# sacs-epfl/decentralized-learning-simulator

Hardware: AMD Instinct MI355X
Metric: device-resident GB/s, N-way weighted model-tensor reduce; 1/2/4/8 MI355X (higher is better)
Workload: dtype f32

## Files before the change

decentralized-learning-simulator_amd/csrc/dispatch.hpp:

```cpp
#pragma once

#include <hip/hip_runtime.h>

#include <algorithm>
#include <cmath>
#include <cstdint>
#include <cstdlib>
#include <cstring>
#include <type_traits>
#include <vector>

#include "dlsim.h"
#include "wreduce_kernels.hpp"
#include "chunk_mean_kernels.hpp"
#include "ab_env.hpp"


namespace dlsim_host __attribute__((visibility("hidden"))) {

int fail(int code, const char* fmt, ...) __attribute__((format(printf, 2, 3)));
int hip_fail(hipError_t e, const char* what);

constexpr int kVpt = 4;
constexpr size_t kBatchSmallBytes = size_t{1} << 20;
// ... 349 lines not shown
                     dim3(dlsim::kBlock), 0, st, s);
  return hipGetLastError();
}

template <class Op, int K, int VPT>
hipError_t launch_batch_fixed(const dlsim::BatchSlots& s, int n, unsigned blocks, hipStream_t st) {
  if constexpr (K > max_fixed_fan_in<Op>()) {
    return launch_batch_nf<Op, 0, VPT>(s, blocks, st);
  } else {
    if (n == K) return launch_batch_nf<Op, K, VPT>(s, blocks, st);
    return launch_batch_fixed<Op, K + 1, VPT>(s, n, blocks, st);
  }
}

template <class Op>
hipError_t launch_batch(const int* fan_in, const size_t* in_off, const void* const* in, const float* w,
                        const float* divs, void* const* outs, const size_t* nelem, int t0, int t1,
                        hipStream_t st) {
  dlsim::BatchSlots s;
  std::memset(&s, 0, sizeof(s));
  const int vpt = batch_vpt<Op>(nelem, t0, t1);
  const size_t tile = static_cast<size_t>(dlsim::kBlock) * vpt;
  uint32_t blocks = 0;
  int ptrs = 0;
  bool uniform = true;
  for (int t = t0; t < t1; ++t) {
    const int k = t - t0;
    const size_t nvec = nelem[t] / Op::E;
    s.out[k] = outs[t];
    s.nvec[k] = nvec;
    s.nelem[k] = nelem[t];
    s.block_start[k] = blocks - static_cast<uint32_t>(k);
    s.ptr_off[k] = static_cast<uint32_t>(ptrs);
    s.fan_in[k] = static_cast<uint32_t>(fan_in[t]);
    s.div[k] = divs ? divs[t] : 1.0f;
    for (int i = 0; i < fan_in[t]; ++i) {
      s.p[ptrs + i] = in[in_off[t] + i];
      s.w[ptrs + i] = w[in_off[t] + i];
    }
    ptrs += fan_in[t];
    blocks += static_cast<uint32_t>(nvec / tile + 1);
    uniform = uniform && fan_in[t] == fan_in[t0];
  }
  s.ntasks = t1 - t0;
  s.block_start[t1 - t0] = blocks - static_cast<uint32_t>(t1 - t0);
  if (vpt == 1) {
    if (uniform) return launch_batch_fixed<Op, 1, 1>(s, fan_in[t0], blocks, st);
    return launch_batch_nf<Op, 0, 1>(s, blocks, st);
  }
  if (uniform) return launch_batch_fixed<Op, 1, 4>(s, fan_in[t0], blocks, st);
  return launch_batch_nf<Op, 0, 4>(s, blocks, st);
}

template <class Op>
int run_batched(int b, const int* fan_in, const void* const* in, const float* w, void* const* outs,
                const size_t* nelem, hipStream_t st, const float* divs = nullptr) {
  std::vector<size_t> off(static_cast<size_t>(b) + 1, 0);
  for (int t = 0; t < b; ++t) off[t + 1] = off[t] + static_cast<size_t>(fan_in[t]);
  if (cross_task_overlap(b, fan_in, in, outs, nelem, Op::kBytes)) {
    for (int t = 0; t < b; ++t) {
      int rc = run<Op>(in + off[t], fan_in[t], w + off[t], outs[t], nelem[t], st, divs ? divs[t] : 1.0f);
      if (rc != DLSIM_OK) return rc;
    }
    return DLSIM_OK;
  }
  auto batchable = [&](int t) {
    if (nelem[t] == 0 || fan_in[t] > 16) return false;
    if (nelem[t] * Op::kBytes > kMaxLaunchOutBytes) return false;
    if (use_defer<Op>(fan_in[t], nelem[t])) return false;
    if (!aligned16(outs[t])) return false;
    for (int i = 0; i < fan_in[t]; ++i)
      if (!aligned16(in[off[t] + i])) return false;
    return true;
  };
  std::vector<int> group;
  for (int t = 0; t < b; ++t) {
    if (batchable(t)) {
      group.push_back(t);
      continue;
    }
    if (nelem[t] == 0) continue;
    int rc = run<Op>(in + off[t], fan_in[t], w + off[t], outs[t], nelem[t], st, divs ? divs[t] : 1.0f);
    if (rc != DLSIM_OK) return rc;
  }
  std::vector<const void*> ins;
  std::vector<float> ws, dv;
  std::vector<void*> os;
  std::vector<size_t> ne, ioff;
  std::vector<int> fi;
  for (int t : group) {
    ioff.push_back(ins.size());
    for (int i = 0; i < fan_in[t]; ++i) {
      ins.push_back(in[off[t] + i]);
      ws.push_back(w[off[t] + i]);
    }
    os.push_back(outs[t]);
    ne.push_back(nelem[t]);
    fi.push_back(fan_in[t]);
    dv.push_back(divs ? divs[t] : 1.0f);
  }
  const int g = static_cast<int>(group.size());
  const size_t tile1 = dlsim::kBlock;
  int t0 = 0;
  while (t0 < g) {
    int t1 = t0, ptrs = 0;
    uint64_t blocks = 0;
    while (t1 < g && t1 - t0 < dlsim::kBatchMaxTasks && ptrs + fi[t1] <= dlsim::kBatchMaxPtrs &&
           blocks + ne[t1] / Op::E / tile1 + 1 < 0x7fffffffull) {
      ptrs += fi[t1];
      blocks += ne[t1] / Op::E / tile1 + 1;
      ++t1;
    }
    hipError_t e = launch_batch<Op>(fi.data(), ioff.data(), ins.data(), ws.data(), dv.data(), os.data(),
                                    ne.data(), t0, t1, st);
    if (e != hipSuccess) return hip_fail(e, "batched kernel launch");
    t0 = t1;
  }
  return DLSIM_OK;
}

struct TableLayout {
  size_t tasks_off, map_off, ptrs_off, w_off, bytes;
  uint32_t nblocks;
  int vpt;
};

inline size_t round8(size_t x) { return (x + 7) / 8 * 8; }

template <class Op>
// ... 50 lines not shown
    const size_t total = nelem[t] * Op::kBytes;
    if (fan_in[t] > DLSIM_MAX_FUSED_INPUTS || total > kMaxLaunchOutBytes || !aligned16(outs[t]))
      return fail(DLSIM_E_ARG, "task %d cannot be table-batched (fan-in <= %d, 16-B aligned, < 2 GiB)", t,
                  DLSIM_MAX_FUSED_INPUTS);
    const uint32_t nb = task_blocks<Op>(nelem[t], L.vpt);
    tasks[t].out = outs[t];
    tasks[t].nvec = nelem[t] / Op::E;
    tasks[t].nelem = nelem[t];
    tasks[t].block_start = blk - 1;
    tasks[t].ptr_off = off;
    tasks[t].fan_in = static_cast<uint32_t>(fan_in[t]);
    map[t] = static_cast<uint32_t>(t);
    for (uint32_t k = 0; k + 1 < nb; ++k) map[blk + k] = static_cast<uint32_t>(t);
    for (int i = 0; i < fan_in[t]; ++i) {
      if (!aligned16(in[off + i]))
        return fail(DLSIM_E_ARG, "task %d input %d is not 16-byte aligned", t, i);
      ptrs[off + i] = in[off + i];
      ws[off + i] = w[off + i];
    }
    blk += nb - 1;
    off += static_cast<uint32_t>(fan_in[t]);
    uniform = uniform && fan_in[t] == fan_in[0];
  }
  h->uniform_fan_in = uniform ? static_cast<uint32_t>(fan_in[0]) : 0u;
  return DLSIM_OK;
}

template <class Op, int NF, int VPT>
hipError_t launch_table_nf(const void* d_table, uint32_t blocks, hipStream_t st) {
  hipLaunchKernelGGL((dlsim::k_wreduce_batch_table<Op, NF, group_size<Op>(), VPT, kNT, store_policy<Op>(),
                                                    kBatchWave<Op, VPT>>),
                     dim3(blocks), dim3(dlsim::kBlock), 0, st, static_cast<const unsigned char*>(d_table));
  return hipGetLastError();
}

template <class Op, int K, int VPT>
hipError_t launch_table_fixed(const void* d_table, int n, uint32_t blocks, hipStream_t st) {
  if constexpr (K > max_fixed_fan_in<Op>()) {
    return launch_table_nf<Op, 0, VPT>(d_table, blocks, st);
  } else {
    if (n == K) return launch_table_nf<Op, K, VPT>(d_table, blocks, st);
    return launch_table_fixed<Op, K + 1, VPT>(d_table, n, blocks, st);
  }
}

template <class Op>
int table_launch(const void* h_table, const void* d_table, hipStream_t st) {
  const auto* h = static_cast<const dlsim::BatchTableHeader*>(h_table);
  if (h->ntasks == 0) return DLSIM_OK;
  if (h->vpt != 1 && h->vpt != 4)
    return fail(DLSIM_E_ARG, "not a table written by dlsim_batch_table_fill (vectors per lane %u)", h->vpt);
  const int n = static_cast<int>(h->uniform_fan_in);
  hipError_t e;
  if (h->vpt == 1)
    e = n ? launch_table_fixed<Op, 1, 1>(d_table, n, h->nblocks, st) : launch_table_nf<Op, 0, 1>(d_table, h->nblocks, st);
  else
    e = n ? launch_table_fixed<Op, 1, 4>(d_table, n, h->nblocks, st) : launch_table_nf<Op, 0, 4>(d_table, h->nblocks, st);
  if (e != hipSuccess) return hip_fail(e, "table batch launch");
  return DLSIM_OK;
}


inline size_t chunk_mean_ilp_begin(int m, size_t n, int threads, size_t esz = 4, size_t vw = 8) {
  if (n <= 1) return 0;
  const size_t rnd = 128 / esz;
  size_t b = 0, e = n;
  if (!(static_cast<unsigned long long>(m) * n < 32768ULL || threads <= 1)) {
    const size_t tp = static_cast<size_t>(threads) < n ? static_cast<size_t>(threads) : n;
    const size_t cs = (n + tp - 1) / tp;
    for (size_t t = 0; t < tp; ++t) {
      size_t tb = t * cs;
      if (tb >= n) break;
      size_t te = tb + cs < n ? tb + cs : n;
      tb -= tb % rnd;
      if (te != n) te -= te % rnd;
      if (tb < te) {
        b = tb;
        e = te;
      }
    }
  }
  const size_t s1 = e - b;
  return b + (s1 >= vw ? s1 / (4 * vw) * (4 * vw) : s1 / 4 * 4);
}

using CmDefault = dlsim::CmShape<4, true, 8>;
using CmFewRows = dlsim::CmShape<4, true, 4>;
constexpr int kCmFewRowsMax = 6;

constexpr int kCmDeferRMax = 32, kCmDeferU = kDeferU, kCmDeferMinRows = 16;
inline bool chunk_defer_on() {
  static const bool on = [] {
    const char* e = dlsim::ab_getenv("DLSIM_CHUNK_DEFER");
    return !(e && e[0] == '0');
  }();
  return on;
}
inline int chunk_defer_min_m() {
  static const int k = [] {
    const char* e = dlsim::ab_getenv("DLSIM_CHUNK_DEFER_MIN_M");
    return e ? std::atoi(e) : kCmDeferMinRows;
  }();
  return k;
}
constexpr int kCmFixedMinM = 4, kCmFixedMaxM = 15;
inline bool chunk_defer_fixed_on() {
// ... 307 lines not shown
```

decentralized-learning-simulator_amd/csrc/dlsim_abi.hip:

```cpp
#include <hip/hip_runtime.h>

#include <algorithm>
#include <cstdarg>
#include <cstdio>
#include <cstdint>
#include <cstdlib>
#include <cstring>
#include <mutex>
#include <string>
#include <thread>
#include <vector>

#include "abi_common.hpp"
#include "dispatch.hpp"
#include "fanin_checks.hpp"

#include "host_pack.hpp"

namespace dlsim_host __attribute__((visibility("hidden"))) {

template <class F>
int with_policy(int dtype, int mode, F&& f) {
  const bool fast = mode == DLSIM_FAST;
  if (dtype == DLSIM_F32) return fast ? f(dlsim::F32Fast{}) : f(dlsim::F32Exact{});
// ... 1436 lines not shown
            : nullptr;
  }
  if (prev >= 0 && prev != device) (void)hipSetDevice(prev);
  if (!out) return nullptr;
  std::lock_guard<std::mutex> lk(g_pool_mu);
  if (out != p) g_realigned.emplace_back(out, p);
  (contig ? g_pool_contig : g_pool_fallback) += 1;
  g_pool_live += nbytes;
  return out;
}

void dlsim_pool_free(void* d_ptr, size_t nbytes, int device, void* ) {
  if (!d_ptr) return;
  void* base = d_ptr;
  {
    std::lock_guard<std::mutex> lk(g_pool_mu);
    for (size_t i = 0; i < g_realigned.size(); ++i) {
      if (g_realigned[i].first == d_ptr) {
        base = g_realigned[i].second;
        g_realigned.erase(g_realigned.begin() + static_cast<long>(i));
        break;
      }
    }
    g_pool_live -= std::min<unsigned long long>(g_pool_live, nbytes);
  }
  int prev = -1;
  (void)hipGetDevice(&prev);
  if (prev != device) (void)hipSetDevice(device);
  (void)hipFree(base);
  if (prev >= 0 && prev != device) (void)hipSetDevice(prev);
}

void dlsim_pool_stats(unsigned long long* contiguous, unsigned long long* fallback, unsigned long long* live_bytes) {
  std::lock_guard<std::mutex> lk(g_pool_mu);
  if (contiguous) *contiguous = g_pool_contig;
  if (fallback) *fallback = g_pool_fallback;
  if (live_bytes) *live_bytes = g_pool_live;
}

const char* dlsim_last_error(void) { return g_err.c_str(); }

const char* dlsim_kernel_name(int n, size_t n_elems, int dtype, int mode) {
  if (dtype != DLSIM_F32 && dtype != DLSIM_BF16 && dtype != DLSIM_F16) return "";
  if (mode == -1) return with_mean_policy_name(dtype, n, n_elems);
  if (mode != DLSIM_EXACT && mode != DLSIM_FAST) return "";
  const char* name = "";
  with_policy(dtype, mode, [&](auto op) {
    name = kernel_name<decltype(op)>(n, n_elems);
    return 0;
  });
  return name;
}

int dlsim_version(void) { return (1 << 16) | 1; }

}
```

decentralized-learning-simulator_amd/csrc/wreduce_kernels.hpp:

```cpp
#pragma once

#include <hip/hip_runtime.h>
#include <stdint.h>

#include <type_traits>

#pragma clang fp contract(off)

namespace dlsim {

constexpr int kBlock = 256;

typedef uint32_t u32x4 __attribute__((ext_vector_type(4)));
typedef float f32x2 __attribute__((ext_vector_type(2)));
typedef __bf16 bf16x2 __attribute__((ext_vector_type(2)));

__device__ __forceinline__ float bf16_round(float f) {
  uint32_t u = __float_as_uint(f);
  if ((u & 0x7fffffffu) > 0x7f800000u) return __uint_as_float(0x7fc00000u);
  u += 0x7fffu + ((u >> 16) & 1u);
  return __uint_as_float(u & 0xffff0000u);
}

__device__ __forceinline__ void bf16_round2(float& a0, float& a1) {
// ... 673 lines not shown
      defer_rows<Op, S, NF, G, RMAX, U, STP>(*ks, n, o, base, R, nvec);
    }
  } else {
    for (int r = 0; r < R; ++r)
      reduce_tile<Op, S, NF, G, 1, 1, true, STP, kDeferBlock>(s, NF > 0 ? NF : n, o,
                                                              base + static_cast<size_t>(r) * kDeferBlock, nvec);
  }
  if (blockIdx.x == 0) {
    const size_t j = nvec * Op::E + threadIdx.x;
    if (j < nelem) fold_scalar<Op, S>(s, NF > 0 ? NF : n, out, j);
  }
}

template <class Op, class S, int NF, int G, int RMAX, int U, int STP, int RC = 0>
__global__ __launch_bounds__(kDeferBlock) void k_wreduce_defer(const S s, int n, int Rrt, void* __restrict__ out,
                                                               size_t nvec, size_t nelem) {
  defer_body<Op, S, NF, G, RMAX, U, STP, RC>(s, n, Rrt, out, nvec, nelem);
}

template <class Op, class S, int NF, int G, int RMAX, int U, int STP, int RC = 0>
__global__ __launch_bounds__(kDeferBlock) void k_wreduce_defer_pre(size_t nvec, void* __restrict__ out,
                                                                   const void* q0, const void* q1, const void* q2,
                                                                   const void* q3, const void* q4, const S s, int n,
                                                                   int Rrt, size_t nelem) {
  static_assert(NF > 0, "fixed fan-in");
  const PreSlots<S> ps{{q0, q1, q2, q3, q4}, s};
  defer_body<Op, PreSlots<S>, NF, G, RMAX, U, STP, RC>(ps, n, Rrt, out, nvec, nelem);
}

constexpr int kBatchMaxTasks = 32;
constexpr int kBatchMaxPtrs = 192;

struct BatchSlots {
  const void* p[kBatchMaxPtrs];
  float w[kBatchMaxPtrs];
  void* out[kBatchMaxTasks];
  size_t nvec[kBatchMaxTasks];
  size_t nelem[kBatchMaxTasks];
  float div[kBatchMaxTasks];
  uint32_t block_start[kBatchMaxTasks + 1];
  uint32_t ptr_off[kBatchMaxTasks];
  uint32_t fan_in[kBatchMaxTasks];
  int ntasks;
};
static_assert(sizeof(BatchSlots) <= 4096, "kernel arguments");

__device__ __forceinline__ int batch_find_task(const BatchSlots& s, uint32_t f) {
  int t = 0;
#pragma unroll
  for (int j = 1; j < kBatchMaxTasks; ++j) t += (j < s.ntasks && f >= s.block_start[j]) ? 1 : 0;
  return t;
}

struct TaskArgs {
  const BatchSlots& b;
  int off;
  float d;
  __device__ const void* ptr(int i) const { return b.p[off + i]; }
  __device__ float wt(int i) const { return b.w[off + i]; }
  __device__ float divisor() const { return d; }
};

template <class Op, int NF, int G, int VPT, int NT, int STP, bool WAVEMAP = false>
__global__ __launch_bounds__(kBlock) void k_wreduce_batch(const BatchSlots s) {
  const uint32_t bid = blockIdx.x;
  int t = 0;
  uint32_t local = 0;
  if (bid < static_cast<uint32_t>(s.ntasks)) {
    t = static_cast<int>(bid);
  } else {
    const uint32_t f = bid - static_cast<uint32_t>(s.ntasks);
    t = batch_find_task(s, f);
    local = f - s.block_start[t] + 1;
  }
  const TaskArgs a{s, static_cast<int>(s.ptr_off[t]), s.div[t]};
  const int n = NF > 0 ? NF : static_cast<int>(s.fan_in[t]);
  const size_t nvec = s.nvec[t];
  constexpr size_t kTile = static_cast<size_t>(kBlock) * VPT;
  const size_t full = nvec / kTile;
  const OutRef o = make_out<STP>(s.out[t], nvec);
  if (local == 0) {
    if (full * kTile < nvec)
      reduce_tile<Op, TaskArgs, NF, G, VPT, NT, true, STP>(a, n, o, full * kTile + threadIdx.x, nvec);
    const size_t j = nvec * Op::E + threadIdx.x;
    if (j < s.nelem[t]) fold_scalar<Op, TaskArgs>(a, n, s.out[t], j);
    return;
  }
  if constexpr (WAVEMAP) {
    const size_t lane_off = (threadIdx.x >> 6) * 64 * VPT + (threadIdx.x & 63);
    reduce_tile<Op, TaskArgs, NF, G, VPT, NT, false, STP, 64>(a, n, o, (local - 1) * kTile + lane_off, nvec);
  } else {
    reduce_tile<Op, TaskArgs, NF, G, VPT, NT, false, STP>(a, n, o, (local - 1) * kTile + threadIdx.x, nvec);
  }
}

struct BatchTableHeader {
  uint32_t ntasks;
  uint32_t nblocks;
  uint32_t uniform_fan_in;
  uint32_t vpt;
  uint64_t tasks_off;
  uint64_t map_off;
  uint64_t ptrs_off;
  uint64_t w_off;
};

struct BatchTaskDesc {
  void* out;
  uint64_t nvec;
  uint64_t nelem;
  uint32_t block_start;
  uint32_t ptr_off;
  uint32_t fan_in;
  uint32_t reserved;
};

struct TableArgs {
  const void* const* p;
  const float* w;
  __device__ const void* ptr(int i) const { return p[i]; }
  __device__ float wt(int i) const { return w[i]; }
  __device__ float divisor() const { return 1.0f; }
};

template <class Op, int NF, int G, int VPT, int NT, int STP, bool WAVEMAP = false>
__global__ __launch_bounds__(kBlock) void k_wreduce_batch_table(const unsigned char* __restrict__ table) {
  const BatchTableHeader* h = reinterpret_cast<const BatchTableHeader*>(table);
  const uint32_t* map = reinterpret_cast<const uint32_t*>(table + h->map_off);
  const uint32_t t = map[blockIdx.x];
  const BatchTaskDesc d = reinterpret_cast<const BatchTaskDesc*>(table + h->tasks_off)[t];
  const TableArgs a{reinterpret_cast<const void* const*>(table + h->ptrs_off) + d.ptr_off,
                    reinterpret_cast<const float*>(table + h->w_off) + d.ptr_off};
  const int n = NF > 0 ? NF : static_cast<int>(d.fan_in);
  const size_t nvec = d.nvec;
  constexpr size_t kTile = static_cast<size_t>(kBlock) * VPT;
  const size_t full = nvec / kTile;
  const OutRef o = make_out<STP>(d.out, nvec);
  const uint32_t local = blockIdx.x < h->ntasks ? 0u : blockIdx.x - d.block_start;
  if (local == 0) {
    if (full * kTile < nvec)
      reduce_tile<Op, TableArgs, NF, G, VPT, NT, true, STP>(a, n, o, full * kTile + threadIdx.x, nvec);
    const size_t j = nvec * Op::E + threadIdx.x;
    if (j < d.nelem) fold_scalar<Op, TableArgs>(a, n, d.out, j);
    return;
  }
// ... 99 lines not shown
```

decentralized-learning-simulator_amd/dasklearn_amd/_native.py:

```python
from __future__ import annotations

import ctypes
import os
import threading
from typing import Optional, Sequence

import numpy as np

LIB_DIR = os.path.join(os.path.dirname(os.path.abspath(__file__)), "lib")
LIB_PATH = os.path.join(LIB_DIR, "libdlsim_hip.so")

DLSIM_F32 = 0
DLSIM_BF16 = 1
DLSIM_F16 = 2
DLSIM_F64 = 3
DLSIM_EXACT = 0
DLSIM_FAST = 1
MAX_FUSED_INPUTS = 128
DLSIM_E_ARG = -1
DLSIM_E_RCCL = -4
DLSIM_E_PEER = -5
DLSIM_E_DISAGREE = -6
DLSIM_GATHER_NONE = 0
DLSIM_GATHER_BCAST = 1
# ... 10 lines not shown
    "dlsim_wreduce_f64",
    "dlsim_wreduce_tensors",
    "dlsim_wreduce_batched",
    "dlsim_batch_table_bytes",
    "dlsim_batch_table_fill",
    "dlsim_batch_table_launch",
    "dlsim_mean",
    "dlsim_mean_batched",
    "dlsim_chunk_mean_batched",
    "dlsim_chunk_mean_ilp_begin",
    "dlsim_chunk_mean_plan",
    "dlsim_rccl_bind",
    "dlsim_wreduce_sharded",
    "dlsim_wreduce_sharded_f64",
    "dlsim_wreduce_mixed",
    "dlsim_sgd_step",
    "dlsim_sgd_step_tensors",
    "dlsim_sgd_momentum_step",
    "dlsim_sgd_momentum_step_tensors",
    "dlsim_robust_reduce",
    "dlsim_robust_reduce_tensors",
    "dlsim_robust_reduce_batched",
    "dlsim_robust_batch_geometry",
    "dlsim_robust_reduce_tensors_batched",
    "dlsim_robust_nearest_reduce",
    "dlsim_robust_nearest_reduce_tensors",
    "dlsim_pairwise_sqdist",
    "dlsim_pairwise_sqdist_tensors",
    "dlsim_pairdist_geometry",
    "dlsim_pairwise_sqdist_batched",
    "dlsim_pairdist_batch_geometry",
    "dlsim_wreduce_dist_batched",
    "dlsim_reducedist_batch_geometry",
    "dlsim_wreduce_dist",
    "dlsim_wreduce_dist_tensors",
    "dlsim_reducedist_geometry",
    "dlsim_device_alloc",
    "dlsim_device_free",
    "dlsim_pool_alloc",
    "dlsim_pool_free",
    "dlsim_pool_stats",
    "dlsim_sharded_plan_create",
    "dlsim_sharded_plan_run",
    "dlsim_sharded_plan_run_f64",
    "dlsim_sharded_plan_destroy",
    "dlsim_host_wreduce",
    "dlsim_host_wreduce_zc",
    "dlsim_host_wreduce_resident",
    "dlsim_host_chunk_mean",
    "dlsim_host_pack",
    "dlsim_shard_range",
    "dlsim_probe_pattern",
    "dlsim_kernel_name",
    "dlsim_last_error",
    "dlsim_version",
)

_lib = None
_lock = threading.Lock()


class ChunkLaunch(ctypes.Structure):
    _fields_ = [("form", ctypes.c_int), ("mf", ctypes.c_int), ("rows", ctypes.c_int), ("bpt", ctypes.c_int),
                ("grid", ctypes.c_uint), ("ntasks", ctypes.c_int), ("first_task", ctypes.c_int)]


CHUNK_FORMS = ("tiled_few", "tiled", "table", "defer_rf4", "defer_rf8", "defer_m")


class DlsimError(RuntimeError):

    def __init__(self, fn: str, rc: int, msg: str):
        super().__init__(f"{fn} failed (rc={rc}): {msg}")
        self.rc = rc


def load() -> ctypes.CDLL:
    global _lib
    if _lib is not None:
        return _lib
    with _lock:
        if _lib is not None:
            return _lib
        if not os.path.exists(LIB_PATH):
            raise ImportError(
                f"HIP extension not built: {LIB_PATH} is missing. Run "
                "`python -c 'import __graft_entry__ as g; g.build()'` at the repo root.")
        lib = ctypes.CDLL(LIB_PATH)
        vp, sz, i = ctypes.c_void_p, ctypes.c_size_t, ctypes.c_int
        lib.dlsim_wreduce.argtypes = [ctypes.POINTER(vp), i, ctypes.POINTER(ctypes.c_float), vp,
                                      sz, i, i, vp]
        lib.dlsim_wreduce.restype = i
        lib.dlsim_wreduce_f64.argtypes = [ctypes.POINTER(vp), i, ctypes.POINTER(ctypes.c_double), vp, sz, i, vp]
        lib.dlsim_wreduce_f64.restype = i
        lib.dlsim_wreduce_tensors.argtypes = [ctypes.POINTER(vp), i, i, ctypes.POINTER(sz),
                                              ctypes.POINTER(ctypes.c_float), ctypes.POINTER(vp),
                                              i, i, vp]
        lib.dlsim_wreduce_tensors.restype = i
        lib.dlsim_wreduce_batched.argtypes = [i, ctypes.POINTER(i), ctypes.POINTER(vp),
                                              ctypes.POINTER(ctypes.c_float), ctypes.POINTER(vp),
                                              ctypes.POINTER(sz), i, i, vp]
        lib.dlsim_wreduce_batched.restype = i
        lib.dlsim_batch_table_bytes.argtypes = [i, ctypes.POINTER(i), ctypes.POINTER(sz), i,
                                                ctypes.POINTER(sz)]
        lib.dlsim_batch_table_bytes.restype = i
        lib.dlsim_batch_table_fill.argtypes = [i, ctypes.POINTER(i), ctypes.POINTER(vp),
# ... 68 lines not shown
                                                                                        dbl, i, vp]
        lib.dlsim_sgd_momentum_step_tensors.restype = i
        lib.dlsim_robust_reduce.argtypes = [ctypes.POINTER(vp), i, i, i, vp, sz, i, vp]
        lib.dlsim_robust_reduce.restype = i
        lib.dlsim_robust_reduce_tensors.argtypes = [ctypes.POINTER(vp), i, i, ctypes.POINTER(sz), ctypes.POINTER(sz),
                                                    i, i, vp, i, vp]
        lib.dlsim_robust_reduce_tensors.restype = i
        lib.dlsim_robust_reduce_batched.argtypes = [i, ctypes.POINTER(i), ctypes.POINTER(vp), ctypes.POINTER(i),
                                                    ctypes.POINTER(i), ctypes.POINTER(vp), ctypes.POINTER(sz), i, vp]
        lib.dlsim_robust_reduce_batched.restype = i
        lib.dlsim_robust_batch_geometry.argtypes = [i, i, ctypes.POINTER(sz), ctypes.POINTER(i), ctypes.POINTER(i)]
        lib.dlsim_robust_batch_geometry.restype = i
        lib.dlsim_robust_reduce_tensors_batched.argtypes = lib.dlsim_robust_reduce_tensors.argtypes
        lib.dlsim_robust_reduce_tensors_batched.restype = i
        lib.dlsim_robust_nearest_reduce.argtypes = [ctypes.POINTER(vp), i, i, vp, sz, i, vp]
        lib.dlsim_robust_nearest_reduce.restype = i
        lib.dlsim_robust_nearest_reduce_tensors.argtypes = [ctypes.POINTER(vp), i, i, ctypes.POINTER(sz),
                                                            ctypes.POINTER(sz), i, vp, i, vp]
        lib.dlsim_robust_nearest_reduce_tensors.restype = i
        lib.dlsim_pairwise_sqdist.argtypes = [ctypes.POINTER(vp), i, sz, i, vp, i, vp]
        lib.dlsim_pairwise_sqdist.restype = i
        lib.dlsim_pairwise_sqdist_tensors.argtypes = [ctypes.POINTER(vp), i, i, ctypes.POINTER(sz), i, vp, i, vp]
        lib.dlsim_pairwise_sqdist_tensors.restype = i
        lib.dlsim_pairdist_geometry.argtypes = [i, i, sz, ctypes.POINTER(sz), ctypes.POINTER(ctypes.c_uint)]
        lib.dlsim_pairdist_geometry.restype = i
        lib.dlsim_pairwise_sqdist_batched.argtypes = [i, ctypes.POINTER(i), ctypes.POINTER(i), ctypes.POINTER(vp),
                                                      ctypes.POINTER(sz), i, ctypes.POINTER(vp), i, vp]
        lib.dlsim_pairwise_sqdist_batched.restype = i
        lib.dlsim_pairdist_batch_geometry.argtypes = [i, i, ctypes.POINTER(i), ctypes.POINTER(i)]
        lib.dlsim_pairdist_batch_geometry.restype = i
        dp = ctypes.POINTER(ctypes.c_double)
        lib.dlsim_wreduce_dist.argtypes = [ctypes.POINTER(vp), i, dp, vp, sz, i, vp, i, vp]
        lib.dlsim_wreduce_dist.restype = i
        lib.dlsim_wreduce_dist_tensors.argtypes = [ctypes.POINTER(vp), i, i, ctypes.POINTER(sz), ctypes.POINTER(sz),
                                                   dp, vp, i, vp, i, vp]
        lib.dlsim_wreduce_dist_tensors.restype = i
        lib.dlsim_reducedist_geometry.argtypes = [i, i, sz, ctypes.POINTER(sz), ctypes.POINTER(ctypes.c_uint)]
        lib.dlsim_reducedist_geometry.restype = i
        lib.dlsim_wreduce_dist_batched.argtypes = [i, ctypes.POINTER(i), ctypes.POINTER(i), ctypes.POINTER(vp),
                                                   ctypes.POINTER(sz), ctypes.POINTER(sz), dp, ctypes.POINTER(vp), i,
                                                   ctypes.POINTER(vp), i, vp]
        lib.dlsim_wreduce_dist_batched.restype = i
        lib.dlsim_reducedist_batch_geometry.argtypes = [i, i, ctypes.POINTER(i), ctypes.POINTER(i)]
        lib.dlsim_reducedist_batch_geometry.restype = i
        lib.dlsim_device_alloc.argtypes = [sz, i, ctypes.POINTER(vp), ctypes.POINTER(i)]
        lib.dlsim_device_alloc.restype = i
        lib.dlsim_device_free.argtypes = [vp]
        lib.dlsim_device_free.restype = i
        u64p = ctypes.POINTER(ctypes.c_ulonglong)
        lib.dlsim_pool_stats.argtypes = [u64p, u64p, u64p]
        lib.dlsim_pool_stats.restype = None
        lib.dlsim_kernel_name.argtypes = [i, sz, i, i]
        lib.dlsim_kernel_name.restype = ctypes.c_char_p
        lib.dlsim_last_error.argtypes = []
        lib.dlsim_last_error.restype = ctypes.c_char_p
        lib.dlsim_version.argtypes = []
        lib.dlsim_version.restype = i
        _lib = lib
        return lib


def kernel_name(n: int, numel: int, torch_dtype, mode: Optional[int] = DLSIM_EXACT) -> str:
    return load().dlsim_kernel_name(n, numel, dtype_code(torch_dtype), -1 if mode is None else mode).decode()


def _check(fn: str, rc: int) -> None:
    if rc != 0:
        msg = load().dlsim_last_error().decode(errors="replace")
        raise DlsimError(fn, rc, msg)


def version() -> int:
    return load().dlsim_version()


def shard_range(n_elems: int, world: int, rank: int, align_elems: int = 64):
    lib = load()
    b, e = ctypes.c_size_t(0), ctypes.c_size_t(0)
    _check("dlsim_shard_range",
           lib.dlsim_shard_range(n_elems, world, rank, align_elems, ctypes.byref(b), ctypes.byref(e)))
    return b.value, e.value


def fp32_weights(weights: Sequence[float]) -> np.ndarray:
    return np.asarray([float(w) for w in weights], dtype=np.float64).astype(np.float32)


def f64_weights(weights: Sequence[float]) -> np.ndarray:
    return np.asarray([float(w) for w in weights], dtype=np.float64)


def weights_for_dtype(weights: Sequence[float], torch_dtype) -> np.ndarray:
    import torch
    return f64_weights(weights) if torch_dtype == torch.float64 else fp32_weights(weights)


def dtype_code(torch_dtype, single_task: bool = False) -> int:
    import torch
    if torch_dtype == torch.float32:
        return DLSIM_F32
    if torch_dtype == torch.bfloat16:
        return DLSIM_BF16
    if torch_dtype == torch.float16:
        return DLSIM_F16
    if torch_dtype == torch.float64:
        if single_task:
            return DLSIM_F64
        raise TypeError("float64 parameters are reduced one task at a time (dlsim_wreduce_f64); "
                        "this entry point takes float32, bfloat16 and float16")
    raise TypeError(f"aggregation supports float32, bfloat16, float16 and float64 parameters, got {torch_dtype}")


def _stream_handle(device, stream) -> Optional[int]:
    import torch
    if stream is not None:
        return stream.cuda_stream
# ... 1127 lines not shown
```

include/dlsim.h:

```cpp
#ifndef DLSIM_H_
#define DLSIM_H_

#include <stddef.h>
#include <stdint.h>

#ifdef __cplusplus
extern "C" {
#endif

enum dlsim_dtype {
  DLSIM_F32 = 0,
  DLSIM_BF16 = 1,
  DLSIM_F16 = 2,
  DLSIM_F64 = 3
};

enum dlsim_mode {
  DLSIM_EXACT = 0,
  DLSIM_FAST = 1
};

#define DLSIM_OK 0
#define DLSIM_E_ARG (-1)
#define DLSIM_E_DTYPE (-2)
// ... 147 lines not shown
int dlsim_robust_batch_geometry(int n, int dtype, size_t* tile_elems, int* max_tasks, int* max_ptrs);

int dlsim_robust_reduce_tensors_batched(const void* const* d_inputs, int n, int t, const size_t* n_elems,
                                        const size_t* out_off_bytes, int lo, int hi, void* d_out, int dtype,
                                        void* stream);

int dlsim_robust_nearest_reduce(const void* const* d_inputs, int n, int keep, void* d_out, size_t n_elems, int dtype,
                                void* stream);

int dlsim_robust_nearest_reduce_tensors(const void* const* d_inputs, int n, int t, const size_t* n_elems,
                                        const size_t* out_off_bytes, int keep, void* d_out, int dtype, void* stream);

#define DLSIM_MAX_PAIRDIST_INPUTS 32
int dlsim_pairwise_sqdist(const void* const* d_inputs, int n, size_t n_elems, int dtype, double* d_d2, int accumulate,
                          void* stream);

int dlsim_pairwise_sqdist_tensors(const void* const* d_inputs, int n, int t, const size_t* n_elems, int dtype,
                                  double* d_d2, int accumulate, void* stream);

int dlsim_pairdist_geometry(int n, int dtype, size_t n_elems, size_t* tile_elems, unsigned* blocks);

#define DLSIM_PAIRDIST_BATCH_MAX_SEGMENTS 32
#define DLSIM_PAIRDIST_BATCH_MAX_PTRS 192
int dlsim_pairwise_sqdist_batched(int b, const int* fan_in, const int* n_tensors, const void* const* d_inputs,
                                  const size_t* n_elems, int dtype, double* const* d_d2, int accumulate, void* stream);

int dlsim_pairdist_batch_geometry(int n, int dtype, int* max_segments, int* max_ptrs);

#define DLSIM_MAX_REDUCEDIST_INPUTS 32
int dlsim_wreduce_dist(const void* const* d_inputs, int n, const double* h_weights, void* d_out, size_t n_elems,
                       int dtype, double* d_d2, int accumulate, void* stream);

int dlsim_wreduce_dist_tensors(const void* const* d_inputs, int n, int t, const size_t* n_elems,
                               const size_t* out_off_bytes, const double* h_weights, void* d_out, int dtype,
                               double* d_d2, int accumulate, void* stream);

int dlsim_reducedist_geometry(int n, int dtype, size_t n_elems, size_t* tile_elems, unsigned* blocks);

#define DLSIM_REDUCEDIST_BATCH_MAX_SEGMENTS 32
int dlsim_wreduce_dist_batched(int b, const int* fan_in, const int* n_tensors, const void* const* d_inputs,
                               const size_t* n_elems, const size_t* out_off_bytes, const double* h_weights,
                               void* const* d_out, int dtype, double* const* d_d2, int accumulate, void* stream);

int dlsim_reducedist_batch_geometry(int n, int dtype, int* max_segments, int* max_ptrs);

#define DLSIM_ALLOC_CONTIGUOUS 1
int dlsim_device_alloc(size_t nbytes, int flags, void** d_out, int* contiguous);
int dlsim_device_free(void* d_ptr);

void* dlsim_pool_alloc(size_t nbytes, int device, void* stream);
void dlsim_pool_free(void* d_ptr, size_t nbytes, int device, void* stream);
void dlsim_pool_stats(unsigned long long* contiguous, unsigned long long* fallback, unsigned long long* live_bytes);

const char* dlsim_kernel_name(int n, size_t n_elems, int dtype, int mode);

const char* dlsim_last_error(void);

int dlsim_version(void);

#ifdef __cplusplus
}
#endif

#endif
```

Measured before the change: 6655.

## Add batched deferred-row reduce kernel for mid-size f32 exact multi-task batches

```diff
diff --git a/decentralized-learning-simulator_amd/csrc/dispatch.hpp b/decentralized-learning-simulator_amd/csrc/dispatch.hpp
--- a/decentralized-learning-simulator_amd/csrc/dispatch.hpp
+++ b/decentralized-learning-simulator_amd/csrc/dispatch.hpp
@@ -425,6 +425,70 @@
   return launch_batch_nf<Op, 0, 4>(s, blocks, st);
 }
 
+constexpr int kBatchDeferMinFanIn = 3, kBatchDeferMaxFanIn = 10, kBatchDeferRMin = 4, kBatchDeferRMax = 24;
+constexpr size_t kBatchDeferMinTaskBytes = 4000000;
+inline int batch_defer_switch() {
+  static const int v = [] {
+    const char* e = dlsim::ab_getenv("DLSIM_BATCH_DEFER");
+    return e ? std::atoi(e) : -1;
+  }();
+  return v;
+}
+inline bool batch_defer_forced() { return batch_defer_switch() > 0; }
+template <class Op> bool batch_defer_fan_in(int n) {
+  return std::is_same<Op, dlsim::F32Exact>::value && batch_defer_switch() != 0 && n >= kBatchDeferMinFanIn &&
+         n <= kBatchDeferMaxFanIn;
+}
+template <class Op> bool batch_defer_task_size(int n, size_t nelem) {
+  if (nelem == 0 || nelem * Op::kBytes > kMaxLaunchOutBytes) return false;
+  return batch_defer_forced() || (nelem * Op::kBytes >= kBatchDeferMinTaskBytes && !use_defer<Op>(n, nelem));
+}
+inline size_t batch_defer_blocks(const dlsim::BatchSlots& s, size_t R) {
+  size_t b = 0;
+  for (int t = 0; t < s.ntasks; ++t) {
+    const size_t rows = (s.nvec[t] + dlsim::kDeferBlock - 1) / dlsim::kDeferBlock;
+    b += rows ? (rows + R - 1) / R : 1;
+  }
+  return b;
+}
+inline int batch_defer_rows(const dlsim::BatchSlots& s, size_t cus) {
+  const int sw = batch_defer_switch();
+  if (sw >= kBatchDeferRMin) return std::min(sw, kBatchDeferRMax) & ~1;
+  for (int R = kBatchDeferRMin; R <= kBatchDeferRMax; R += 2)
+    if (batch_defer_blocks(s, static_cast<size_t>(R)) <= cus) return R;
+  int best = kBatchDeferRMax;
+  double best_cost = 1e300;
+  for (int R = kBatchDeferRMax / 2; R <= kBatchDeferRMax; R += 2) {
+    const double w = static_cast<double>(batch_defer_blocks(s, static_cast<size_t>(R))) / static_cast<double>(cus);
+    const double full = std::floor(w), x = w - full;
+    const double cost = R * (full + (x > 0 ? std::max(x, 0.38 + 0.45 * x) : 0.0)) + 0.1 * std::ceil(w);
+    if (cost < best_cost - 1e-9) {
+      best_cost = cost;
+      best = R;
+    }
+  }
+  return best;
+}
+hipError_t launch_batch_defer_f32(const dlsim::BatchSlots& s, int nf, int R, uint32_t bpt, unsigned blocks,
+                                  hipStream_t st);
+unsigned long long batch_defer_launch_count();
+inline hipError_t launch_batch_defer(dlsim::BatchSlots& s, int nf, hipStream_t st) {
+  const int R = batch_defer_rows(s, static_cast<size_t>(device_cus()));
+  uint32_t blocks = 0, bpt = 0;
+  for (int t = 0; t < s.ntasks; ++t) {
+    const size_t rows = (s.nvec[t] + dlsim::kDeferBlock - 1) / dlsim::kDeferBlock;
+    const uint32_t tb = static_cast<uint32_t>(rows ? (rows + R - 1) / R : 1);
+    s.block_start[t] = blocks;
+    s.ptr_off[t] = static_cast<uint32_t>(t * nf);
+    s.fan_in[t] = static_cast<uint32_t>(nf);
+    s.div[t] = 1.0f;
+    bpt = t == 0 ? tb : (bpt == tb ? tb : 0);
+    blocks += tb;
+  }
+  s.block_start[s.ntasks] = blocks;
+  return launch_batch_defer_f32(s, nf, R, bpt, blocks, st);
+}
+
 template <class Op>
 int run_batched(int b, const int* fan_in, const void* const* in, const float* w, void* const* outs,
                 const size_t* nelem, hipStream_t st, const float* divs = nullptr) {
@@ -437,17 +501,48 @@
     }
     return DLSIM_OK;
   }
-  auto batchable = [&](int t) {
-    if (nelem[t] == 0 || fan_in[t] > 16) return false;
-    if (nelem[t] * Op::kBytes > kMaxLaunchOutBytes) return false;
-    if (use_defer<Op>(fan_in[t], nelem[t])) return false;
+  auto aligned = [&](int t) {
     if (!aligned16(outs[t])) return false;
     for (int i = 0; i < fan_in[t]; ++i)
       if (!aligned16(in[off[t] + i])) return false;
     return true;
   };
+  std::vector<char> taken(static_cast<size_t>(b), 0);
+  for (int nf = kBatchDeferMinFanIn; nf <= kBatchDeferMaxFanIn && batch_defer_fan_in<Op>(nf); ++nf) {
+    std::vector<int> cand;
+    for (int t = 0; t < b; ++t)
+      if (fan_in[t] == nf && batch_defer_task_size<Op>(nf, nelem[t]) && aligned(t)) cand.push_back(t);
+    const size_t per = std::min<size_t>(dlsim::kBatchMaxTasks, dlsim::kBatchMaxPtrs / static_cast<size_t>(nf));
+    for (size_t c0 = 0; c0 < cand.size(); c0 += per) {
+      const size_t c1 = std::min(cand.size(), c0 + per);
+      if (c1 - c0 < 2 && !batch_defer_forced()) continue;
+      dlsim::BatchSlots s;
+      std::memset(&s, 0, sizeof(s));
+      for (size_t c = c0; c < c1; ++c) {
+        const int t = cand[c], k = static_cast<int>(c - c0);
+        s.out[k] = outs[t];
+        s.nvec[k] = nelem[t] / Op::E;
+        s.nelem[k] = nelem[t];
+        for (int i = 0; i < nf; ++i) {
+          s.p[k * nf + i] = in[off[t] + i];
+          s.w[k * nf + i] = w[off[t] + i];
+        }
+        taken[static_cast<size_t>(t)] = 1;
+      }
+      s.ntasks = static_cast<int>(c1 - c0);
+      const hipError_t e = launch_batch_defer(s, nf, st);
+      if (e != hipSuccess) return hip_fail(e, "deferred batch launch");
+    }
+  }
+  auto batchable = [&](int t) {
+    if (nelem[t] == 0 || fan_in[t] > 16) return false;
+    if (nelem[t] * Op::kBytes > kMaxLaunchOutBytes) return false;
+    if (use_defer<Op>(fan_in[t], nelem[t])) return false;
+    return aligned(t);
+  };
   std::vector<int> group;
   for (int t = 0; t < b; ++t) {
+    if (taken[static_cast<size_t>(t)]) continue;
     if (batchable(t)) {
       group.push_back(t);
       continue;
@@ -604,6 +699,44 @@
     return fail(DLSIM_E_ARG, "not a table written by dlsim_batch_table_fill (vectors per lane %u)", h->vpt);
   const int n = static_cast<int>(h->uniform_fan_in);
   hipError_t e;
+  const auto* base = static_cast<const unsigned char*>(h_table);
+  const auto* tasks = reinterpret_cast<const dlsim::BatchTaskDesc*>(base + h->tasks_off);
+  const auto* ptrs = reinterpret_cast<const void* const*>(base + h->ptrs_off);
+  const auto* ws = reinterpret_cast<const float*>(base + h->w_off);
+  if (std::is_same<Op, dlsim::F32Exact>::value && batch_defer_switch() < 0) {
+    bool alone = true;
+    for (uint32_t t = 0; t < h->ntasks && alone; ++t)
+      alone = use_defer<Op>(static_cast<int>(tasks[t].fan_in), tasks[t].nelem);
+    if (alone) {
+      for (uint32_t t = 0; t < h->ntasks; ++t) {
+        const int rc = run<Op>(ptrs + tasks[t].ptr_off, static_cast<int>(tasks[t].fan_in), ws + tasks[t].ptr_off,
+                               tasks[t].out, tasks[t].nelem, st);
+        if (rc != DLSIM_OK) return rc;
+      }
+      return DLSIM_OK;
+    }
+  }
+  if (batch_defer_fan_in<Op>(n) && h->ntasks <= static_cast<uint32_t>(dlsim::kBatchMaxTasks) &&
+      h->ntasks * static_cast<uint32_t>(n) <= static_cast<uint32_t>(dlsim::kBatchMaxPtrs) &&
+      (h->ntasks >= 2 || batch_defer_forced())) {
+    bool ok = true;
+    for (uint32_t t = 0; t < h->ntasks && ok; ++t) ok = batch_defer_task_size<Op>(n, tasks[t].nelem);
+    if (ok) {
+      dlsim::BatchSlots s;
+      std::memset(&s, 0, sizeof(s));
+      for (uint32_t t = 0; t < h->ntasks; ++t) {
+        s.out[t] = tasks[t].out;
+        s.nvec[t] = tasks[t].nvec;
+        s.nelem[t] = tasks[t].nelem;
+      }
+      std::memcpy(s.p, ptrs, sizeof(void*) * h->ntasks * static_cast<size_t>(n));
+      std::memcpy(s.w, ws, sizeof(float) * h->ntasks * static_cast<size_t>(n));
+      s.ntasks = static_cast<int>(h->ntasks);
+      e = launch_batch_defer(s, n, st);
+      if (e != hipSuccess) return hip_fail(e, "deferred table batch launch");
+      return DLSIM_OK;
+    }
+  }
   if (h->vpt == 1)
     e = n ? launch_table_fixed<Op, 1, 1>(d_table, n, h->nblocks, st) : launch_table_nf<Op, 0, 1>(d_table, h->nblocks, st);
   else
diff --git a/decentralized-learning-simulator_amd/csrc/dlsim_abi.hip b/decentralized-learning-simulator_amd/csrc/dlsim_abi.hip
--- a/decentralized-learning-simulator_amd/csrc/dlsim_abi.hip
+++ b/decentralized-learning-simulator_amd/csrc/dlsim_abi.hip
@@ -1512,6 +1512,8 @@
   return name;
 }
 
+unsigned long long dlsim_batch_defer_launches(void) { return batch_defer_launch_count(); }
+
 int dlsim_version(void) { return (1 << 16) | 1; }
 
 }
diff --git a/decentralized-learning-simulator_amd/csrc/inst_batch_defer.hip b/decentralized-learning-simulator_amd/csrc/inst_batch_defer.hip
--- /dev/null
+++ b/decentralized-learning-simulator_amd/csrc/inst_batch_defer.hip
@@ -0,0 +1,46 @@
+#include <atomic>
+
+#include "dispatch.hpp"
+
+namespace dlsim_host {
+
+namespace {
+
+std::atomic<unsigned long long> g_launches{0};
+
+template <int NF, int RC>
+hipError_t launch_rc(const dlsim::BatchSlots& s, int R, uint32_t bpt, unsigned blocks, hipStream_t st) {
+  if constexpr (RC > kBatchDeferRMax) {
+    return hipErrorInvalidValue;
+  } else {
+    if (R == RC) {
+      hipLaunchKernelGGL((dlsim::k_wreduce_batch_defer<dlsim::F32Exact, NF, RC, kDeferU, kStore>), dim3(blocks),
+                         dim3(dlsim::kDeferBlock), 0, st, bpt, s);
+      return hipGetLastError();
+    }
+    return launch_rc<NF, RC + kDeferU>(s, R, bpt, blocks, st);
+  }
+}
+
+template <int NF>
+hipError_t launch_nf(const dlsim::BatchSlots& s, int nf, int R, uint32_t bpt, unsigned blocks, hipStream_t st) {
+  if constexpr (NF > kBatchDeferMaxFanIn) {
+    return hipErrorInvalidValue;
+  } else {
+    if (nf == NF) return launch_rc<NF, kBatchDeferRMin>(s, R, bpt, blocks, st);
+    return launch_nf<NF + 1>(s, nf, R, bpt, blocks, st);
+  }
+}
+
+}
+
+hipError_t launch_batch_defer_f32(const dlsim::BatchSlots& s, int nf, int R, uint32_t bpt, unsigned blocks,
+                                  hipStream_t st) {
+  if (blocks == 0 || blocks > 0x7fffffffu) return hipErrorInvalidValue;
+  g_launches.fetch_add(1, std::memory_order_relaxed);
+  return launch_nf<kBatchDeferMinFanIn>(s, nf, R, bpt, blocks, st);
+}
+
+unsigned long long batch_defer_launch_count() { return g_launches.load(std::memory_order_relaxed); }
+
+}
diff --git a/decentralized-learning-simulator_amd/csrc/wreduce_kernels.hpp b/decentralized-learning-simulator_amd/csrc/wreduce_kernels.hpp
--- a/decentralized-learning-simulator_amd/csrc/wreduce_kernels.hpp
+++ b/decentralized-learning-simulator_amd/csrc/wreduce_kernels.hpp
@@ -749,6 +749,19 @@
   return t;
 }
 
+__device__ __forceinline__ int batch_find_task(const BatchSlots& s, uint32_t f, uint32_t* start) {
+  int t = 0;
+  uint32_t st = 0;
+#pragma unroll
+  for (int j = 1; j < kBatchMaxTasks; ++j) {
+    const bool past = j < s.ntasks && f >= s.block_start[j];
+    t += past ? 1 : 0;
+    st = past ? s.block_start[j] : st;
+  }
+  *start = st;
+  return t;
+}
+
 struct TaskArgs {
   const BatchSlots& b;
   int off;
@@ -788,6 +801,51 @@
     reduce_tile<Op, TaskArgs, NF, G, VPT, NT, false, STP, 64>(a, n, o, (local - 1) * kTile + lane_off, nvec);
   } else {
     reduce_tile<Op, TaskArgs, NF, G, VPT, NT, false, STP>(a, n, o, (local - 1) * kTile + threadIdx.x, nvec);
+  }
+}
+
+template <int NF>
+struct FixedSlots {
+  const void* p[NF];
+  float w[NF];
+  __device__ const void* ptr(int i) const { return p[i]; }
+  __device__ float wt(int i) const { return w[i]; }
+  __device__ float divisor() const { return 1.0f; }
+};
+
+template <class Op, int NF, int RC, int U, int STP>
+__global__ __launch_bounds__(kDeferBlock) void k_wreduce_batch_defer(uint32_t bpt, const BatchSlots s) {
+  static_assert(NF > 0 && RC > 0, "fixed fan-in, compiled row count");
+  const uint32_t bid = blockIdx.x;
+  uint32_t t, local;
+  if (bpt) {
+    t = bid / bpt;
+    local = bid - t * bpt;
+  } else {
+    t = static_cast<uint32_t>(batch_find_task(s, bid, &local));
+    local = bid - local;
+  }
+  FixedSlots<NF> a;
+#pragma unroll
+  for (int i = 0; i < NF; ++i) {
+    a.p[i] = s.p[t * NF + i];
+    a.w[i] = s.w[t * NF + i];
+  }
+  const size_t nvec = s.nvec[t];
+  void* out = s.out[t];
+  const OutRef o = make_out<STP>(out, nvec);
+  constexpr size_t span = static_cast<size_t>(kDeferBlock) * RC;
+  const size_t base = static_cast<size_t>(local) * span + threadIdx.x;
+  if (static_cast<size_t>(local + 1) * span <= nvec) {
+    defer_rows_c<Op, FixedSlots<NF>, NF, 8, RC, U, STP>(a, NF, o, base);
+  } else {
+    for (int r = 0; r < RC; ++r)
+      reduce_tile<Op, FixedSlots<NF>, NF, 8, 1, 1, true, STP, kDeferBlock>(
+          a, NF, o, base + static_cast<size_t>(r) * kDeferBlock, nvec);
+  }
+  if (local == 0) {
+    const size_t j = nvec * Op::E + threadIdx.x;
+    if (j < s.nelem[t]) fold_scalar<Op, FixedSlots<NF>>(a, NF, out, j);
   }
 }
 
diff --git a/decentralized-learning-simulator_amd/dasklearn_amd/_native.py b/decentralized-learning-simulator_amd/dasklearn_amd/_native.py
--- a/decentralized-learning-simulator_amd/dasklearn_amd/_native.py
+++ b/decentralized-learning-simulator_amd/dasklearn_amd/_native.py
@@ -86,6 +86,7 @@
     "dlsim_shard_range",
     "dlsim_probe_pattern",
     "dlsim_kernel_name",
+    "dlsim_batch_defer_launches",
     "dlsim_last_error",
     "dlsim_version",
 )
@@ -260,6 +261,8 @@
         lib.dlsim_pool_stats.restype = None
         lib.dlsim_kernel_name.argtypes = [i, sz, i, i]
         lib.dlsim_kernel_name.restype = ctypes.c_char_p
+        lib.dlsim_batch_defer_launches.argtypes = []
+        lib.dlsim_batch_defer_launches.restype = ctypes.c_ulonglong
         lib.dlsim_last_error.argtypes = []
         lib.dlsim_last_error.restype = ctypes.c_char_p
         lib.dlsim_version.argtypes = []
@@ -270,6 +273,10 @@
 
 def kernel_name(n: int, numel: int, torch_dtype, mode: Optional[int] = DLSIM_EXACT) -> str:
     return load().dlsim_kernel_name(n, numel, dtype_code(torch_dtype), -1 if mode is None else mode).decode()
+
+
+def batch_defer_launches() -> int:
+    return int(load().dlsim_batch_defer_launches())
 
 
 def _check(fn: str, rc: int) -> None:
diff --git a/include/dlsim.h b/include/dlsim.h
--- a/include/dlsim.h
+++ b/include/dlsim.h
@@ -223,6 +223,8 @@
 void dlsim_pool_free(void* d_ptr, size_t nbytes, int device, void* stream);
 void dlsim_pool_stats(unsigned long long* contiguous, unsigned long long* fallback, unsigned long long* live_bytes);
 
+unsigned long long dlsim_batch_defer_launches(void);
+
 const char* dlsim_kernel_name(int n, size_t n_elems, int dtype, int mode);
 
 const char* dlsim_last_error(void);
```

Result: no change. 6645 (-0.1%).
